# CIS565-Fall-2014/Project3-Pathtracer

Measured on AMD Instinct MI355X. Metric: ray-bounces/sec, higher is better.
Workload: dtype f32

## Files before the change

### project3-pathtracer_amd/csrc/pt_bounce.h

```cpp
#pragma once
#include <stdlib.h>

#include "pt_internal.h"

namespace pt {
using namespace ptd;

static constexpr uint32_t DEAD = 0xFFFFFFFFu;
#ifndef PT_DEBUG_PAIR
#define PT_DEBUG_PAIR 0
#endif
#ifndef PT_DEBUG_PHASE
#define PT_DEBUG_PHASE 0
#endif
#ifndef PT_DEBUG_BVH
#define PT_DEBUG_BVH 0
#endif
#ifndef PT_DEBUG_SPAN
#define PT_DEBUG_SPAN 0
#endif
static constexpr bool DEBUG_SPAN = PT_DEBUG_SPAN != 0;
#ifndef PT_DEBUG_BOUNDS
#define PT_DEBUG_BOUNDS 0
#endif
// ... 3 lines not shown
static constexpr bool DEBUG_PHASE = PT_DEBUG_PHASE == 1;
static constexpr bool DEBUG_PHASE2 = PT_DEBUG_PHASE == 2;
template <bool FIRST> __device__ __forceinline__ constexpr bool LANE_BUDGET() { return FIRST ? PT_DEBUG_PHASE == 3 : PT_DEBUG_PHASE == 2; }
static constexpr bool DEBUG_BVH = PT_DEBUG_BVH != 0;
static constexpr int MAXSLOT = 16;
static constexpr uint32_t SLOT_SHIFT = 27;
static constexpr uint32_t PIX_MASK = (1u << SLOT_SHIFT) - 1u;

typedef const __attribute__((address_space(4))) uint32_t *const_u32_ptr;
typedef float v4f __attribute__((ext_vector_type(4)));
typedef float v2f __attribute__((ext_vector_type(2)));
template <class V> __device__ __forceinline__ void nt_store(V v, V *p)
{
#if defined(PT_NO_NT)
    *p = v;
#else
    __builtin_nontemporal_store(v, p);
#endif
}
template <class V> __device__ __forceinline__ V nt_load(const V *p)
{
#if defined(PT_NO_NT)
    return *p;
#else
    return __builtin_nontemporal_load(p);
#endif
}

__device__ __forceinline__ bool dbgInRange(const KParams &p, int code, unsigned long long v, unsigned long long lim)
{
    if (!DEBUG_BOUNDS || v < lim) return true;
    if (atomicCAS(&p.st->dbg[0], 0ull, (unsigned long long)code) == 0ull) { p.st->dbg[1] = v; p.st->dbg[2] = lim; p.st->dbg[4] = blockIdx.x; p.st->dbg[5] = threadIdx.x; }
    return false;
}

__device__ __forceinline__ Prim load_prim_scalar(const Prim *prims, int g)
{
    Prim r;
    const_u32_ptr q = (const_u32_ptr)(uintptr_t)(prims + g);
    uint32_t *dst = reinterpret_cast<uint32_t *>(&r);
#pragma unroll
    for (int k = 0; k < 32; ++k) dst[k] = q[k];
    return r;
}

struct PrimPad : Prim { uint32_t pad_lds[4]; };
static_assert(sizeof(PrimPad) == 144, "PrimPad must be 144 B");
template <class PR> __device__ __forceinline__ constexpr uint32_t faceStride() { return (uint32_t)(sizeof(PR) / 16); }

struct Hit {
    f3 p, n;
    uint32_t material;
    uint32_t prim;
    float t;
    bool any;
    uint32_t self_ok;
    unsigned long long dbg0, dbg1;
    unsigned long long dbg2, dbg3;
};

enum { GEOM_SCALAR = 0, GEOM_LDS = 1, GEOM_QUEUE = 2, GEOM_BVH = 3, GEOM_PAIR = 4, GEOM_WALK_PAIR = 5, GEOM_WALK4 = 6,
       GEOM_WALK4G = 7 };

__device__ __forceinline__ bool waveMissesBound(const Prim &P, f3 o, f3 d)
{
    const f3 oc = o - mk(P.cx, P.cy, P.cz);
// ... 1545 lines not shown
                        q = (q < 0.05f) ? 0.05f : ((q > 1.0f) ? 1.0f : q);
                        if (u01_of(minstd_jump(s0, MINSTD_A4)) >= q) alive = false;
                        else T = mk(T.x / q, T.y / q, T.z / q);
                    }
                    if (NEE) pix = (pix & 0x7FFFFFFFu) | (diffuse ? 0x80000000u : 0u);
                    }
                }
            }
        }
        if (NEE) {
            const uint64_t wmask = __ballot(want_shadow);
            if (wmask != 0ull) {
                shadow_count += (uint32_t)__popcll(wmask);
                Hit hs;
                if (MOTION && GEOM == GEOM_PAIR) {
                    hs = nearestHit<GEOM, false, true>(p, s_prims, s_nodes + (PAIR_BOX_BYTES / 16) * p.nG, wq, so, sd, want_shadow, (uint32_t)lane, 0xFFFFFFFFu, mt);
                } else if (MOTION) {
                    hs.any = false; hs.material = 0; hs.prim = 0; hs.t = 0.0f; hs.p = mk(0, 0, 0); hs.n = mk(0, 0, 0);
                    if (want_shadow) hs = nearestHitMotion(p, so, sd, mt);
                } else {
                    hs = nearestHit<GEOM, false>(p, s_prims, (GEOM == GEOM_PAIR) ? s_nodes + (PAIR_BOX_BYTES / 16) * p.nG : s_nodes, wq, so, sd, want_shadow, (uint32_t)lane);
                }
                if (want_shadow && hs.any && hs.prim == lprim) {
                    const float tol = 1e-3f * ((ldist > 1.0f) ? ldist : 1.0f);
                    if (fabsf(hs.t - ldist) <= tol) L = L + Ld;
                }
            }
            if (valid && (L.x != 0.0f || L.y != 0.0f || L.z != 0.0f)) {
                float4 *lp = reinterpret_cast<float4 *>(p.lbuf) + ((size_t)((pix >> SLOT_SHIFT) & (uint32_t)(MAXSLOT - 1)) * npix + (size_t)(pix & PIX_MASK));
                if (!dbgInRange(p, 6, (unsigned long long)((pix >> SLOT_SHIFT) & (uint32_t)(MAXSLOT - 1)) * npix + (pix & PIX_MASK), (unsigned long long)npix * st->nslot)) lp = reinterpret_cast<float4 *>(p.lbuf);
                float4 e = *lp;
                if (__float_as_uint(e.w) != serial) e = make_float4(0.0f, 0.0f, 0.0f, 0.0f);
                *lp = make_float4(e.x + L.x, e.y + L.y, e.z + L.z, __uint_as_float(serial));
            }
        } else if (valid && !alive && (L.x != 0.0f || L.y != 0.0f || L.z != 0.0f)) {
            float4 *lp = reinterpret_cast<float4 *>(p.lbuf) + ((size_t)(pix >> SLOT_SHIFT) * npix + (size_t)(pix & PIX_MASK));
            if (!dbgInRange(p, 7, (unsigned long long)(pix >> SLOT_SHIFT) * npix + (pix & PIX_MASK), (unsigned long long)npix * st->nslot)) lp = reinterpret_cast<float4 *>(p.lbuf);
            nt_store((v4f){L.x, L.y, L.z, __uint_as_float(serial)}, reinterpret_cast<v4f *>(lp));
        }

        const unsigned long long c3 = (DEBUG_PHASE || PT_DEBUG_PHASE == 2 || PT_DEBUG_PHASE == 3) ? __builtin_amdgcn_s_memtime() : 0ull;
        if (DEBUG_PHASE) { ph[0] += c1 - tc0; ph[1] += c2 - c1; ph[2] += c3 - c2; ph[4] += 1; }
        if (LANE_BUDGET<FIRST>()) { ph[0] += c1 - tc0; ph[1] += c2 - c1; ph[2] += c3 - c2; ph[4] += 1; ph5 += h.dbg0 + h.dbg2; ph6 += h.dbg1; }
        if (LANE_BUDGET<FIRST>() && GEOM == GEOM_PAIR) {
            lb_nbsdf = (uint32_t)__popcll(__ballot(did_bsdf));
            const unsigned long long res = (c2 - c1) - h.dbg0 - h.dbg1 - h.dbg2;
            lbud[0] += c1 - tc0;  lbud[1] += (c1 - tc0) * lb_nvalid;
            lbud[2] += h.dbg0;    lbud[3] += h.dbg0 * lb_nvalid;
            lbud[4] += h.dbg2;
            lbud[5] += h.dbg1;    lbud[6] += h.dbg3;
            lbud[7] += res;       lbud[8] += res * lb_nhit;
            lbud[9] += c3 - c2;   lbud[10] += (c3 - c2) * lb_nbsdf;
            lbud[13] += 1;        lbud[14] += lb_nvalid;
        }
        if (RESIDENT) {
            if (valid && !alive) atomicAdd(&s_term[cb], 1u);
            valid = alive;
            lb = (cb + 1u) | (leaves_outside ? ((h.prim + 1u) << 8) : 0u);
            if (DEBUG_PHASE2 && GEOM == GEOM_PAIR) { const unsigned long long c4 = __builtin_amdgcn_s_memtime() - c3; lbud[11] += c4; lbud[12] += c4 * (unsigned long long)__popcll(__ballot(alive)); }
            continue;
        }
        if (last) continue;

        if (COMPACT != 0) {
            const uint64_t mask = __ballot(alive);
            const uint32_t rank = __builtin_amdgcn_mbcnt_hi((uint32_t)(mask >> 32),
                                                            __builtin_amdgcn_mbcnt_lo((uint32_t)mask, 0u));
            const uint32_t wtot = (uint32_t)__popcll(mask);
            uint32_t dst;
            if (COMPACT == 1 || NW == 1) {
                uint32_t b = 0;
// ... 161 lines not shown
```

### project3-pathtracer_amd/csrc/pt_context.hip

```cpp
#include <math.h>
#include <stdarg.h>
#include <stdio.h>
#include <stdlib.h>
#include <string.h>

#include <algorithm>
#include <string>
#include <vector>

#include "pt_internal.h"
#include "pt_scene.h"

#ifndef PT_RESIDENT_DEFAULT
#define PT_RESIDENT_DEFAULT 1
#endif
#ifndef PT_REFILL_MIN_DEFAULT
#define PT_REFILL_MIN_DEFAULT 8
#endif

namespace {
thread_local std::string g_last_error;
}

int pt::fail(int code, const char *fmt, ...)
// ... 54 lines not shown
    pt::KParams kps[PT_MAX_SEQUENCES];
    int nseq = 1;
    hipStream_t seq_stream[PT_MAX_SEQUENCES] = {};
    hipEvent_t seq_acc[PT_MAX_SEQUENCES] = {};
    hipEvent_t seq_fork = nullptr;
    pt::LaunchCfg cfg;
    ptd::Prim *d_prims = nullptr;
    float *d_mats = nullptr;
    float *d_ro_eye = nullptr;
    float *d_face_n = nullptr;
    float *d_box_eye = nullptr;
    std::vector<float> h_box_eye;
    std::vector<ptd::BvhNode> h_bvh;
    std::vector<float> h_boxes;
    uint32_t *d_span_off = nullptr, *d_span_list = nullptr;
    size_t span_off_cap = 0, span_list_cap = 0;
    uint32_t *d_span_mask = nullptr;
    size_t span_mask_cap = 0;
    float *d_box_world = nullptr;
    float *d_slab_n = nullptr;
    pt::LightRec *d_lights = nullptr;
    float *d_knots = nullptr, *d_knot_cam = nullptr;
    int *d_light_tris = nullptr;
    float *d_light_cdf = nullptr;
    ptd::BvhNode *d_bvh = nullptr;
    float *d_bvh4 = nullptr;
    float *d_image_own = nullptr;
    float *d_image_bound = nullptr;
    size_t image_bytes = 0, image_cap = 0;
    void *d_pool = nullptr;
    size_t pool_cap = 0;
    float *d_lbuf = nullptr;
    size_t lbuf_cap = 0;
    unsigned long long batches_stamped = 0;
    int batch = 1;
    pt::IterState *d_state = nullptr;
    bool image_valid = false;

    hipGraph_t graph[PT_MAX_SEQUENCES + 1] = {};
    hipGraphExec_t graph_exec[PT_MAX_SEQUENCES + 1] = {};

    std::vector<std::pair<hipEvent_t, hipEvent_t>> timers;
    double gpu_ms = 0.0;
    unsigned long long bounce_launches = 0;
};

namespace {

void drop_graph(pt_ctx *c)
{
    for (int q = 0; q <= PT_MAX_SEQUENCES; ++q) {
        if (c->graph_exec[q]) { (void)hipGraphExecDestroy(c->graph_exec[q]); c->graph_exec[q] = nullptr; }
        if (c->graph[q]) { (void)hipGraphDestroy(c->graph[q]); c->graph[q] = nullptr; }
    }
}

hipError_t sync_all_streams(pt_ctx *c)
{
    hipError_t first = hipStreamSynchronize(c->stream);
    for (int sq = 1; sq < PT_MAX_SEQUENCES; ++sq)
        if (c->seq_stream[sq]) {
            const hipError_t e = hipStreamSynchronize(c->seq_stream[sq]);
            if (first == hipSuccess) first = e;
        }
    return first;
}
// ... 879 lines not shown
    if (per_cu < 1) return fail(PT_ERR_HIP, "occupancy query failed for workgroup=%d (%s)", cfg.workgroup,
                                hipGetErrorString(hipGetLastError()));
    {
        const long long fit = (160LL * 1024) / ((long long)lds + 1300);
        if (fit >= 1 && per_cu > (int)fit) per_cu = (int)fit;
    }
    int cap = 6 * 256 / cfg.workgroup;
    if (cap < 1) cap = 1;
    if (getenv("PT_MAX_WG_PER_CU") && atoi(getenv("PT_MAX_WG_PER_CU")) > 0) cap = atoi(getenv("PT_MAX_WG_PER_CU"));
    if (per_cu > cap) per_cu = cap;
    int batch = o.batch == 0 ? pt::PT_MAX_BATCH : o.batch;
    while (batch > 1 && (long long)npix * batch > (1LL << 28)) --batch;
    if (npix >= (1 << 27)) return fail(PT_ERR_INVALID, "tile of %d pixels too large (pixel index must fit 27 bits)", npix);
    c->batch = batch;
    k.nslot = batch;
    const long long nrays = (long long)npix * batch;
    const long long want = (nrays + cfg.workgroup - 1) / cfg.workgroup;
    long long grid = (long long)c->cu_count * per_cu;
    if (grid > want) grid = want;
    if (grid < 1) grid = 1;
    cfg.grid = (int)grid;
    if (cfg.resident && !pt::bounce_resident_available(cfg)) cfg.resident = 0;
    cfg.slab = slab_wanted();
    if (!cfg.slab) k.slab_mask = 0u;
    if (getenv("PT_DEBUG_CLOCK"))
        fprintf(stderr, "[ptamd] launch: geom %d, workgroup %d, %zu B LDS, %d workgroups/CU, grid %d, batch %d, resident paths %d (refill at %d free lanes)\n", cfg.geom, cfg.workgroup,
                lds, per_cu, cfg.grid, batch, cfg.resident, k.refill_min);

    int nseq = o.sequences == 0 ? 2 : o.sequences;
    if (o.sequences == 0 && getenv("PT_SEQUENCES") && atoi(getenv("PT_SEQUENCES")) >= 1 && atoi(getenv("PT_SEQUENCES")) <= PT_MAX_SEQUENCES)
        nseq = atoi(getenv("PT_SEQUENCES"));
    c->nseq = nseq;
    const size_t lbuf_bytes = ((size_t)nrays * 4 * sizeof(float) + 255) & ~(size_t)255;

    k.span_mask = nullptr;
    k.span_off = nullptr;
    k.span_list = nullptr;
    const bool spans_ok = k.eye_cull && !(k.lens_radius > 0.0f) && npix / 64 <= (1 << 21);
    const bool want_mask = spans_ok && !cfg.motion && cfg.geom == 4 && k.nG <= 32 && k.ntri == 0 && c->h_box_eye.size() >= (size_t)k.nG * 8;
    const bool want_lists = spans_ok && npix % 64 == 0 && (cfg.geom == 6 || cfg.geom == 7) && c->h_boxes.size() >= (size_t)k.nG * 6 && k.nG <= 65536;
    if (want_mask || want_lists) {
        const int nspan = (npix + 63) / 64;
        const double ex = k.eye[0], ey = k.eye[1], ez = k.eye[2];
        const double eye3[3] = {ex, ey, ez};
        const double vw[3] = {(double)k.M[0] - ex, (double)k.M[1] - ey, (double)k.M[2] - ez};
        auto gpix = [&](uint32_t pl) -> uint32_t {
            if (k.strip_span == 0u) return pl + k.pix_offset;
            const uint32_t j = pl / k.strip_span;
            return pl + k.strip_span * (j * (k.strip_world - 1u) + k.strip_rank);
        };
        auto dirOf = [&](double sx, double sy, double *o3) {
            for (int a = 0; a < 3; ++a) o3[a] = vw[a] + (1.0 - 2.0 * sx) * (double)k.H[a] + (1.0 - 2.0 * sy) * (double)k.V[a];
        };
        double sx_margin, sy_margin;
        {
            double big = 0.0, lh = 0.0, lv = 0.0;
            for (int a = 0; a < 3; ++a) {
                big = std::max(big, fabs(eye3[a]) + fabs(vw[a]) + fabs((double)k.H[a]) + fabs((double)k.V[a]));
                lh += (double)k.H[a] * (double)k.H[a]; lv += (double)k.V[a] * (double)k.V[a];
            }
            const double err = 3.0 * 1.1920929e-7 * big * 1.7320508;
            sx_margin = lh > 0.0 ? err / (2.0 * sqrt(lh)) : 1e30;
            sy_margin = lv > 0.0 ? err / (2.0 * sqrt(lv)) : 1e30;
        }
        const bool ray_grid_ok = sx_margin < 1.0 && sy_margin < 1.0;
        struct Frustum { double nrm[4][3], cc[3], lcc; bool planes_ok, narrow; };
// ... 128 lines not shown
            }
        }
    }

    {
        const long long nw = cfg.workgroup / 64;
        const long long total_waves = (long long)cfg.grid * nw;
        const long long chunks = (nrays + 63) / 64 + pt::NSHARD;
        const long long rounds = (chunks + total_waves - 1) / total_waves;
        long long writers = total_waves;
        if (k.nshard > 1) writers = (total_waves + k.nshard - 1) / k.nshard;
        long long segcap = writers * rounds * 64;
        const long long npad = (nrays + 63) & ~63LL;
        if (k.nshard == 1 || segcap > npad) segcap = npad;
        k.segcap = (uint32_t)segcap;
    }
    const size_t slots = (size_t)k.segcap * (size_t)k.nshard;
    const size_t one = slots * (16 + 16 + 8);
    for (;;) {
        hipError_t e = hipSuccess;
        if (c->lbuf_cap < lbuf_bytes * (size_t)nseq) {
            if (c->d_lbuf) (void)hipFree(c->d_lbuf);
            c->d_lbuf = nullptr; c->lbuf_cap = 0;
            e = hipMalloc((void **)&c->d_lbuf, lbuf_bytes * (size_t)nseq);
            if (e == hipSuccess) {
                c->lbuf_cap = lbuf_bytes * (size_t)nseq;
                HIP_TRY(hipMemsetAsync(c->d_lbuf, 0, c->lbuf_cap, c->stream));
                HIP_TRY(hipStreamSynchronize(c->stream));
                for (uint32_t sq = 0; sq < (uint32_t)PT_MAX_SEQUENCES; ++sq)
                    HIP_TRY(hipMemcpy(&c->d_state[sq].serial, &sq, sizeof sq, hipMemcpyHostToDevice));
                c->batches_stamped = 0;
            } else c->d_lbuf = nullptr;
        }
        if (e == hipSuccess && c->pool_cap < 2 * one * (size_t)nseq) {
            if (c->d_pool) (void)hipFree(c->d_pool);
            c->d_pool = nullptr; c->pool_cap = 0;
            e = hipMalloc(&c->d_pool, 2 * one * (size_t)nseq);
            if (e == hipSuccess) c->pool_cap = 2 * one * (size_t)nseq;
            else c->d_pool = nullptr;
        }
        if (e == hipSuccess) break;
        (void)hipGetLastError();
        if (nseq > 1) { nseq = 1; c->nseq = 1; continue; }
        c->dirty = true;
        return fail(PT_ERR_OOM, "device memory: %zu B of ray pools + %zu B of radiance planes per launch sequence (%s)", 2 * one, lbuf_bytes,
                    hipGetErrorString(e));
    }
    k.lbuf = c->d_lbuf;
    for (int sq = 0; sq < PT_MAX_SEQUENCES; ++sq) {
        pt::KParams &ks = c->kps[sq];
        ks = k;
        if (sq >= nseq) continue;
        for (int q = 0; q < 2; ++q) {
            unsigned char *base = (unsigned char *)c->d_pool + (size_t)(2 * sq + q) * one;
            ks.pool[q].a = (float4 *)base;
            ks.pool[q].b = (float4 *)(base + slots * 16);
            ks.pool[q].c = (float2 *)(base + slots * 32);
        }
        ks.lbuf = (float *)((unsigned char *)c->d_lbuf + (size_t)sq * lbuf_bytes);
        ks.st = c->d_state + sq;
    }
    k = c->kps[0];
    if (getenv("PT_DEBUG_CLOCK")) fprintf(stderr, "[ptamd] launch sequences in flight: %d\n", nseq);

    c->dirty = false;
    return PT_OK;
}

int bounce_launches_per_batch(const pt_ctx *c) { return c->cfg.resident ? 2 : c->kp.depth; }

int book_batch_serials(pt_ctx *c, unsigned long long nb)
{
    static const unsigned long long serial_budget =
        (getenv("PT_SERIAL_BUDGET") && atoll(getenv("PT_SERIAL_BUDGET")) > 0) ? (unsigned long long)atoll(getenv("PT_SERIAL_BUDGET")) : (1ull << 29);
    if (c->batches_stamped + nb > serial_budget) {
        HIP_TRY(sync_all_streams(c));
        HIP_TRY(hipMemset(c->d_lbuf, 0, c->lbuf_cap));
        for (uint32_t sq = 0; sq < (uint32_t)PT_MAX_SEQUENCES; ++sq)
            HIP_TRY(hipMemcpy(&c->d_state[sq].serial, &sq, sizeof sq, hipMemcpyHostToDevice));
        c->batches_stamped = 0;
    }
    c->batches_stamped += nb;
    return PT_OK;
}

int enqueue_batch(pt_ctx *c, hipStream_t s, hipEvent_t *ev, int sq = 0, bool with_accumulate = true)
{
    const pt::KParams &kp = c->kps[sq];
    HIP_TRY(pt::launch_iter_begin(s, kp.st, kp.npix, kp.depth, c->cfg.compact));
    const int launches = bounce_launches_per_batch(c);
    for (int b = 0; b < launches; ++b) {
        if (ev) HIP_TRY(hipEventRecord(ev[2 * b], s));
        HIP_TRY(pt::launch_bounce(s, kp, c->cfg, b));
        if (ev) HIP_TRY(hipEventRecord(ev[2 * b + 1], s));
    }
    if (with_accumulate) HIP_TRY(pt::launch_accumulate(s, kp.image, kp.lbuf, kp.st, kp.npix));
    return PT_OK;
}

void batch_schedule(int iter_count, int batch, int *n, int *q, int *r)
{
    *n = (iter_count + batch - 1) / batch;
    *q = iter_count / *n;
    *r = iter_count % *n;
}

float lerp1(float a, float b, float t) { return a + (b - a) * t; }
pt_vec3 lerp3(pt_vec3 a, pt_vec3 b, float t) { return {lerp1(a.x, b.x, t), lerp1(a.y, b.y, t), lerp1(a.z, b.z, t)}; }

void drop_slices(pt_ctx *c)
{
    for (pt_ctx *k : c->slice_ctx) pt_destroy(k);
    c->slice_ctx.clear();
}

int build_slices(pt_ctx *c)
{
    if (!c->motion_dirty) return PT_OK;
    drop_slices(c);
    const int n = c->motion_slices;
    for (int k = 0; k < n; ++k) {
        pt_ctx *ch = nullptr;
        int rc = pt_create(c->device, &ch);
        if (rc != PT_OK) return rc;
        c->slice_ctx.push_back(ch);
        const float t = ((float)k + 0.5f) / (float)n;
        std::vector<pt_static_geom> g = c->geoms;
        for (size_t i = 0; i < g.size(); ++i) {
            const pt_static_geom &a = c->geoms[i], &b = c->geoms_next[i];
// ... 17 lines not shown
                while (a1 < c->tri_geom.size() && c->tri_geom[a1] == c->tri_geom[a0]) ++a1;
                ms.push_back(pt_mesh{c->tri_geom[a0], (int)(a1 - a0), c->tri_obj.data() + 9 * a0});
                a0 = a1;
            }
            rc = pt_set_meshes(ch, ms.data(), (int)ms.size());
        }
        if (rc == PT_OK) rc = pt_set_camera(ch, &cam);
        if (rc != PT_OK) return rc;
    }
    c->motion_dirty = false;
    return PT_OK;
}

int render_batch_ordered(pt_ctx *c, hipStream_t ss, int iter_first, int count, hipEvent_t wait_ev, hipEvent_t done_ev)
{
    int rc = configure(c);
    if (rc != PT_OK) return rc;
    if (count < 1 || count > c->batch) return fail(PT_ERR_INVALID, "render_batch_ordered: %d iterations (batch %d)", count, c->batch);
    rc = book_batch_serials(c, 1ull);
    if (rc != PT_OK) return rc;
    if (c->opt.use_graph && !c->graph_exec[0]) {
        HIP_TRY(hipStreamBeginCapture(ss, hipStreamCaptureModeThreadLocal));
        rc = enqueue_batch(c, ss, nullptr, 0, false);
        hipError_t ce = hipStreamEndCapture(ss, &c->graph[0]);
        if (rc != PT_OK) { drop_graph(c); return rc; }
        if (ce != hipSuccess) { drop_graph(c); return fail(PT_ERR_HIP, "hipStreamEndCapture: %s", hipGetErrorString(ce)); }
        HIP_TRY(hipGraphInstantiate(&c->graph_exec[0], c->graph[0], nullptr, nullptr, 0));
    }
    HIP_TRY(pt::launch_iter_set(ss, c->d_state, (uint32_t)iter_first, (uint32_t)count, 0u, 0u, 1u));
    if (c->opt.use_graph) HIP_TRY(hipGraphLaunch(c->graph_exec[0], ss));
    else { rc = enqueue_batch(c, ss, nullptr, 0, false); if (rc != PT_OK) return rc; }
    if (wait_ev) HIP_TRY(hipStreamWaitEvent(ss, wait_ev, 0));
    const pt::KParams &ks = c->kps[0];
    HIP_TRY(pt::launch_accumulate(ss, ks.image, ks.lbuf, ks.st, ks.npix));
    HIP_TRY(pt::launch_iter_fold(ss, c->d_state, c->kp.depth));
    if (done_ev) HIP_TRY(hipEventRecord(done_ev, ss));
    c->bounce_launches += (unsigned long long)bounce_launches_per_batch(c);
    c->image_valid = true;
    return PT_OK;
}

}

extern "C" {

const char *pt_last_error(void) { return g_last_error.c_str(); }
const char *pt_version(void) { return "ptamd 0.1 (gfx950, abi 2)"; }
int pt_abi_version(void) { return PT_ABI_VERSION; }
size_t pt_options_size(void) { return sizeof(pt_options); }

int pt_strip_local_rows(int height, int strip_rows, int world, int rank)
{
    if (height < 1 || strip_rows < 1 || world < 1 || rank < 0 || rank >= world) return 0;
    const long long nstrips = ((long long)height + strip_rows - 1) / strip_rows;
    long long rows = 0;
    for (long long k = rank; k < nstrips; k += world) {
        const long long left = (long long)height - k * strip_rows;
        rows += left < strip_rows ? left : strip_rows;
    }
    return (int)rows;
}

int pt_strip_global_row(int strip_rows, int world, int rank, int local_row)
{
    if (strip_rows < 1 || world < 1 || rank < 0 || rank >= world || local_row < 0) return -1;
    const int j = local_row / strip_rows, w = local_row % strip_rows;
    return (j * world + rank) * strip_rows + w;
// ... 55 lines not shown
            pt_destroy(c);
            return fail(PT_ERR_HIP, "cannot initialise the iteration state");
        }
    *out = c;
    return PT_OK;
}

void pt_destroy(pt_ctx *c)
{
    if (!c) return;
    drop_slices(c);
    (void)hipSetDevice(c->device);
    if (c->stream) (void)sync_all_streams(c);
    drop_graph(c);
    for (auto &t : c->timers) { (void)hipEventDestroy(t.first); (void)hipEventDestroy(t.second); }
    if (c->d_prims) (void)hipFree(c->d_prims);
    if (c->d_mats) (void)hipFree(c->d_mats);
    if (c->d_ro_eye) (void)hipFree(c->d_ro_eye);
    if (c->d_face_n) (void)hipFree(c->d_face_n);
    if (c->d_box_eye) (void)hipFree(c->d_box_eye);
    if (c->d_span_mask) (void)hipFree(c->d_span_mask);
    if (c->d_box_world) (void)hipFree(c->d_box_world);
    if (c->d_slab_n) (void)hipFree(c->d_slab_n);
    if (c->d_lights) (void)hipFree(c->d_lights);
    if (c->d_light_tris) (void)hipFree(c->d_light_tris);
    if (c->d_light_cdf) (void)hipFree(c->d_light_cdf);
    if (c->d_knots) (void)hipFree(c->d_knots);
    if (c->d_knot_cam) (void)hipFree(c->d_knot_cam);
    if (c->d_bvh) (void)hipFree(c->d_bvh);
    if (c->d_bvh4) (void)hipFree(c->d_bvh4);
    if (c->d_image_own) (void)hipFree(c->d_image_own);
    if (c->d_pool) (void)hipFree(c->d_pool);
    if (c->d_lbuf) (void)hipFree(c->d_lbuf);
    if (c->d_state) (void)hipFree(c->d_state);
    if (c->d_span_off) (void)hipFree(c->d_span_off);
    if (c->d_span_list) (void)hipFree(c->d_span_list);
    for (int q = 1; q < PT_MAX_SEQUENCES; ++q)
        if (c->seq_stream[q]) { (void)hipStreamSynchronize(c->seq_stream[q]); (void)hipStreamDestroy(c->seq_stream[q]); }
    for (int q = 0; q < PT_MAX_SEQUENCES; ++q)
        if (c->seq_acc[q]) (void)hipEventDestroy(c->seq_acc[q]);
    if (c->seq_fork) (void)hipEventDestroy(c->seq_fork);
    if (c->own_stream) (void)hipStreamDestroy(c->own_stream);
    delete c;
}

int pt_set_options(pt_ctx *c, const pt_options *o)
{
    if (!c || !o) return fail(PT_ERR_INVALID, "pt_set_options: NULL argument");
    if (o->depth < 1 || o->depth > PT_MAX_DEPTH) return fail(PT_ERR_INVALID, "depth %d not in 1..%d", o->depth, PT_MAX_DEPTH);
    const int wg = o->workgroup;
    if (!(wg == 0 || wg == 64 || wg == 128 || wg == 256 || wg == 512 || wg == 1024))
        return fail(PT_ERR_INVALID, "workgroup %d not one of 0,64,128,256,512,1024", wg);
    if (o->geom_path < 0 || o->geom_path > 8) return fail(PT_ERR_INVALID, "geom_path %d not in 0..8", o->geom_path);
    if (o->row_begin < 0 || o->row_end < o->row_begin) return fail(PT_ERR_INVALID, "tile rows [%d,%d)", o->row_begin, o->row_end);
    if (o->strip_rows < 0 || (o->strip_rows > 0 && (o->strip_world < 1 || o->strip_rank < 0 || o->strip_rank >= o->strip_world)))
        return fail(PT_ERR_INVALID, "strips: rows %d, rank %d of %d", o->strip_rows, o->strip_rank, o->strip_world);
    if (o->strip_rows > 0 && (o->row_begin != 0 || o->row_end != 0))
        return fail(PT_ERR_INVALID, "strip tiles and a row band [%d,%d) exclude each other", o->row_begin, o->row_end);
    if (o->batch < 0 || o->batch > pt::PT_MAX_BATCH) return fail(PT_ERR_INVALID, "batch %d not in 0..%d", o->batch, pt::PT_MAX_BATCH);
    if (o->compaction < 0 || o->compaction > 2) return fail(PT_ERR_INVALID, "compaction %d not 0, 1 or 2", o->compaction);
    if (o->direct_light < 0 || o->direct_light > 1) return fail(PT_ERR_INVALID, "direct_light %d not 0 or 1", o->direct_light);
    if (o->absorption < 0 || o->absorption > 1) return fail(PT_ERR_INVALID, "absorption %d not 0 or 1", o->absorption);
    if (o->scatter < 0 || o->scatter > 1) return fail(PT_ERR_INVALID, "scatter %d not 0 or 1", o->scatter);
    if (!(o->lens_radius >= 0.0f) || (o->lens_radius > 0.0f && !(o->focal_distance > 0.0f)))
        return fail(PT_ERR_INVALID, "lens radius %g / focal distance %g", (double)o->lens_radius, (double)o->focal_distance);
    if (o->motion_per_ray < 0 || o->motion_per_ray > 1) return fail(PT_ERR_INVALID, "motion_per_ray %d not 0 or 1", o->motion_per_ray);
// ... 260 lines not shown
            if (ce != hipSuccess) { drop_graph(c); return fail(PT_ERR_HIP, "hipStreamEndCapture: %s", hipGetErrorString(ce)); }
            HIP_TRY(hipGraphInstantiate(&c->graph_exec[gs], c->graph[gs], nullptr, nullptr, 0));
        }
    }
    rc = book_batch_serials(c, (unsigned long long)nb);
    if (rc != PT_OK) return rc;
    if (c->timers.size() >= 1024) { rc = fold_timers(c); if (rc != PT_OK) return rc; }
    hipEvent_t e0, e1;
    HIP_TRY(hipEventCreateWithFlags(&e0, hipEventDisableSystemFence));
    HIP_TRY(hipEventCreateWithFlags(&e1, hipEventDisableSystemFence));
    c->timers.emplace_back(e0, e1);
    HIP_TRY(hipEventRecord(e0, s));

    auto forked = [&]() -> int {
        if (nseq > 1) {
            HIP_TRY(hipEventRecord(c->seq_fork, s));
            for (int sq = 1; sq < nseq; ++sq) HIP_TRY(hipStreamWaitEvent(c->seq_stream[sq], c->seq_fork, 0));
        }
        for (int sq = 0; sq < nseq; ++sq)
            HIP_TRY(pt::launch_iter_set(c->seq_stream[sq], c->d_state + sq, (uint32_t)iter_first, (uint32_t)q, (uint32_t)r, (uint32_t)sq, (uint32_t)nseq));
        for (int i = 0; i < nb; ++i) {
            const int sq = i % nseq;
            hipStream_t ss = c->seq_stream[sq];
            if (c->opt.use_graph) {
                const int gs = own_acc ? sq : PT_MAX_SEQUENCES;
                HIP_TRY(hipGraphLaunch(c->graph_exec[gs], ss));
            } else {
                const int rc2 = enqueue_batch(c, ss, nullptr, sq, !own_acc);
                if (rc2 != PT_OK) return rc2;
            }
            if (own_acc) {
                if (i > 0) HIP_TRY(hipStreamWaitEvent(ss, c->seq_acc[(i - 1) % nseq], 0));
                const pt::KParams &ks = c->kps[sq];
                HIP_TRY(pt::launch_accumulate(ss, ks.image, ks.lbuf, ks.st, ks.npix));
                HIP_TRY(hipEventRecord(c->seq_acc[sq], ss));
            }
        }
        for (int sq = 0; sq < nseq; ++sq) HIP_TRY(pt::launch_iter_fold(c->seq_stream[sq], c->d_state + sq, c->kp.depth));
        if (nseq > 1) {
            for (int sq = 1; sq < nseq; ++sq) {
                HIP_TRY(hipEventRecord(c->seq_acc[sq], c->seq_stream[sq]));
                HIP_TRY(hipStreamWaitEvent(s, c->seq_acc[sq], 0));
            }
        }
        HIP_TRY(hipEventRecord(e1, s));
        return PT_OK;
    };
    rc = forked();
    if (rc != PT_OK) {
        (void)sync_all_streams(c);
        c->image_valid = false;
        return rc;
    }
    c->bounce_launches += (unsigned long long)nb * (unsigned long long)bounce_launches_per_batch(c);
    c->image_valid = true;
    return PT_OK;
}

int pt_get_launch_info(pt_ctx *c, pt_launch_info *out)
{
    if (!c || !out) return fail(PT_ERR_INVALID, "pt_get_launch_info: NULL argument");
    int rc = configure(c);
    if (rc != PT_OK) return rc;
    memset(out, 0, sizeof *out);
    out->geom_path = c->cfg.geom + 1;
    out->workgroup = c->cfg.workgroup;
    out->grid = c->cfg.grid;
// ... 231 lines not shown
```

### project3-pathtracer_amd/csrc/pt_internal.h

```cpp
#pragma once
#include <hip/hip_runtime.h>
#include <stdint.h>

#include "../../include/pt_abi.h"
#include "pt_device.h"

namespace pt {

struct RayPool {
    float4 *a;
    float4 *b;
    float2 *c;
};

static constexpr int NSHARD = 32;
static constexpr int PT_MAX_BATCH = 16;
static constexpr int CNT_STRIDE = 32;
__host__ __device__ constexpr int cnt_index(int bounce, int shard) { return (bounce * NSHARD + shard) * CNT_STRIDE; }

struct IterState {
    uint32_t iter;
    uint32_t nslot;
    uint32_t sched_q, sched_r, sched_j;
    uint32_t sched_first, sched_stride;
// ... 18 lines not shown
    float lens_radius, focal_distance;
    int W;
    int row_begin;
    int npix;
    uint32_t pix_offset;
    int nG, nM;
    int depth;
    int rr_start;
    uint32_t seed;
    const ptd::Prim *prims;
    const ptd::BvhNode *bvh;
    int nnodes;
    const float *bvh4;
    int nnodes4;
    int wdepth;
    int ntri;
    int nbig;
    int big[16];
    const float *face_n;
    const float *ro_eye;
    int eye_cull;
    const float *box_world;
    const float *box_eye;
    const float *slab_n;
    uint32_t slab_mask;
    const uint32_t *span_off;
    const uint32_t *span_list;
    const uint32_t *span_mask;
    const float *mats;
    float *image;
    int cull;
    int nslot;
    float *lbuf;
    int nshard;
    uint32_t segcap;
    IterState *st;
    RayPool pool[2];
    uint32_t strip_span;
    uint32_t strip_rows, strip_world, strip_rank;
    uint32_t strip_magic;
    uint32_t strip_shift;
    uint32_t w_magic;
    uint32_t w_shift;
    int absorption;
    int scatter;
    int nlights;
    const LightRec *lights;
    const int *light_tris;
    const float *light_cdf;
    int ngeoms;
    const float *knots;
    const float *knot_cam;
    int nknots;
    float tan_x, tan_y;
    int refill_min;
};

struct LaunchCfg {
    int workgroup;
    int grid;
    int geom;
    int compact;
    int nee;
    int media;
    int motion;
    int resident;
    int slab;
};

hipError_t launch_iter_set(hipStream_t s, IterState *st, uint32_t iter_first, uint32_t q, uint32_t r, uint32_t j0, uint32_t stride);
hipError_t launch_iter_begin(hipStream_t s, IterState *st, int npix, int depth, int compact);
hipError_t launch_accumulate(hipStream_t s, float *image, const float *lbuf, const IterState *st, int npix);
hipError_t launch_iter_fold(hipStream_t s, IterState *st, int depth);
hipError_t launch_bounce(hipStream_t s, const KParams &p, const LaunchCfg &cfg, int bounce);
hipError_t launch_send_image_to_pbo(hipStream_t s, pt_uchar4 *pbo, const float *image, int npix);
hipError_t launch_selftest_math(hipStream_t s, unsigned long long *out3);
hipError_t launch_device_kat(hipStream_t s, int op, const float *in, float *out, int n_out);
int fail(int code, const char *fmt, ...) __attribute__((format(printf, 2, 3)));

size_t bounce_lds_bytes(const KParams &p, const LaunchCfg &cfg);
int bounce_max_blocks_per_cu(const KParams &p, const LaunchCfg &cfg);
bool bounce_resident_available(const LaunchCfg &cfg);

}
```

### project3-pathtracer_amd/csrc/pt_kernels.hip

```cpp
#include <stdlib.h>

#include <algorithm>

#include "pt_bounce.h"

namespace pt {

__global__ __launch_bounds__(256) void k_selftest_math(unsigned long long *out)
{
    const uint64_t stride = (uint64_t)gridDim.x * 256u;
    unsigned long long bad0 = 0, bad1 = 0, bad2 = 0;
    for (uint64_t i = (uint64_t)blockIdx.x * 256u + threadIdx.x; i < (1ull << 32); i += stride) {
        const float x = __uint_as_float((uint32_t)i);
        const float a = sqrtf(x), b = sqrt_rn(x);
        if (__float_as_uint(a) != __float_as_uint(b) && !(a != a && b != b)) bad0++;
        const float c = 1.0f / x, d = rcp_rn(x);
        if (__float_as_uint(c) != __float_as_uint(d) && !(c != c && d != d)) bad1++;
        const float e = 1.0f / sqrtf(x), f = rsqrt_rn(x), g = rsqrt_near_one(x);
        if (__float_as_uint(e) != __float_as_uint(f) && !(e != e && f != f)) bad2++;
        if (__float_as_uint(e) != __float_as_uint(g) && !(e != e && g != g)) bad2++;
        const uint32_t sd = (uint32_t)i, md = sd % 2147483647u;
        if (minstd_seed(sd) != (md == 0u ? 1u : md)) bad2++;
    }
    if (bad0) atomicAdd(&out[0], bad0);
// ... 95 lines not shown
    st->nslot = 0u;
    st->sched_q = q;
    st->sched_r = r;
    st->sched_j = j0;
    st->sched_first = iter_first;
    st->sched_stride = stride;
}

__global__ void k_iter_begin(IterState *st, uint32_t npix, int depth, int compact)
{
    const int b = threadIdx.x;
    const uint32_t j = st->sched_j;
    const uint32_t nslot = st->sched_q + (j < st->sched_r ? 1u : 0u);
    const uint32_t iter = st->sched_first + j * st->sched_q + (j < st->sched_r ? j : st->sched_r);
    __syncthreads();
    if (b <= depth) {
        unsigned long long sum = 0;
        for (int sh = 0; sh < NSHARD; ++sh) {
            sum += st->counts[cnt_index(b, sh)];
            st->counts[cnt_index(b, sh)] = (b == 0 && sh == 0 && compact) ? npix * nslot : 0u;
        }
        if (b < depth) st->live_in[b] += sum;
    }
    if (b < NSHARD) st->draw[b * CNT_STRIDE] = 0u;
    if (b == 0) {
        st->serial += (uint32_t)PT_MAX_SEQUENCES;
        st->iter = iter;
        st->nslot = nslot;
        st->sched_j = j + st->sched_stride;
        st->iterations += nslot;
    }
}

__global__ __launch_bounds__(256) void k_accumulate(float *image, const float4 *lbuf, const IterState *st, int npix)
{
    const uint32_t iter0 = st->iter, serial = st->serial;
    const int nslot = (int)st->nslot;
    for (int i = blockIdx.x * 256 + threadIdx.x; i < npix; i += gridDim.x * 256) {
        float r = image[3 * i], g = image[3 * i + 1], b = image[3 * i + 2];
        float4 L[PT_MAX_BATCH];
#pragma unroll
        for (int k = 0; k < PT_MAX_BATCH; ++k)
            if (k < nslot) {
                const v4f e = __builtin_nontemporal_load(reinterpret_cast<const v4f *>(lbuf + (size_t)k * (size_t)npix + (size_t)i));
                L[k] = make_float4(e.x, e.y, e.z, e.w);
            }
#pragma unroll
        for (int k = 0; k < PT_MAX_BATCH; ++k) {
            if (k < nslot) {
                const bool have = __float_as_uint(L[k].w) == serial;
                const float lr = have ? L[k].x : 0.0f, lg = have ? L[k].y : 0.0f, lb = have ? L[k].z : 0.0f;
                const uint32_t it = iter0 + (uint32_t)k;
                const float fi = (float)it, fim1 = (float)(it - 1u);
                r = (it == 1u) ? lr : (r * fim1 + lr) / fi;
                g = (it == 1u) ? lg : (g * fim1 + lg) / fi;
                b = (it == 1u) ? lb : (b * fim1 + lb) / fi;
            }
        }
        image[3 * i] = r;
        image[3 * i + 1] = g;
        image[3 * i + 2] = b;
    }
}

__global__ void k_iter_fold(IterState *st, int depth)
{
    const int b = threadIdx.x;
    if (b <= depth) {
        unsigned long long sum = 0;
        for (int sh = 0; sh < NSHARD; ++sh) {
            sum += st->counts[cnt_index(b, sh)];
            st->counts[cnt_index(b, sh)] = 0u;
        }
        if (b < depth) st->live_in[b] += sum;
    }
}

__global__ __launch_bounds__(256) void k_send_image_to_pbo(pt_uchar4 *pbo, const float *image, int npix)
{
    for (int i = blockIdx.x * 256 + threadIdx.x; i < npix; i += gridDim.x * 256) {
        float r = image[3 * i] * 255.0f, g = image[3 * i + 1] * 255.0f, b = image[3 * i + 2] * 255.0f;
        if (r > 255) r = 255;
        if (g > 255) g = 255;
        if (b > 255) b = 255;
        pt_uchar4 o;
        o.x = (unsigned char)r;
        o.y = (unsigned char)g;
        o.z = (unsigned char)b;
        o.w = 0;
        pbo[i] = o;
    }
// ... 59 lines not shown
            hipFuncSetAttribute(f0, hipFuncAttributeMaxDynamicSharedMemorySize, (int)lds) != hipSuccess)
            return 0;
    }
    if (hipOccupancyMaxActiveBlocksPerMultiprocessor(&nb, fn, cfg.workgroup, bounce_lds_bytes(p, cfg)) != hipSuccess)
        return 0;
    return nb;
}

hipError_t launch_bounce(hipStream_t s, const KParams &p, const LaunchCfg &cfg, int bounce)
{
    LaunchCfg lc = cfg;
    if (bounce == 0) lc.resident = 0;
    const void *fn = select_bounce(lc, bounce == 0);
    if (!fn) return hipErrorInvalidValue;
    KParams pc = p;
    int b = bounce;
    void *args[] = {(void *)&pc, (void *)&b};
    return hipLaunchKernel(fn, dim3((unsigned)cfg.grid), dim3((unsigned)cfg.workgroup), args,
                           bounce_lds_bytes(p, lc), s);
}

hipError_t launch_iter_set(hipStream_t s, IterState *st, uint32_t iter_first, uint32_t q, uint32_t r, uint32_t j0, uint32_t stride)
{
    hipLaunchKernelGGL(k_iter_set, dim3(1), dim3(1), 0, s, st, iter_first, q, r, j0, stride);
    return hipGetLastError();
}

hipError_t launch_iter_begin(hipStream_t s, IterState *st, int npix, int depth, int compact)
{
    hipLaunchKernelGGL(k_iter_begin, dim3(1), dim3(128), 0, s, st, (uint32_t)npix, depth, compact != 0 ? 1 : 0);
    return hipGetLastError();
}

hipError_t launch_accumulate(hipStream_t s, float *image, const float *lbuf, const IterState *st, int npix)
{
    int grid = (npix + 255) / 256;
    if (grid > 16384) grid = 16384;
    if (grid < 1) grid = 1;
    hipLaunchKernelGGL(k_accumulate, dim3(grid), dim3(256), 0, s, image, reinterpret_cast<const float4 *>(lbuf), st, npix);
    return hipGetLastError();
}

hipError_t launch_iter_fold(hipStream_t s, IterState *st, int depth)
{
    hipLaunchKernelGGL(k_iter_fold, dim3(1), dim3(128), 0, s, st, depth);
    return hipGetLastError();
}

hipError_t launch_send_image_to_pbo(hipStream_t s, pt_uchar4 *pbo, const float *image, int npix)
{
    int grid = (npix + 255) / 256;
    if (grid > 4096) grid = 4096;
    if (grid < 1) grid = 1;
    hipLaunchKernelGGL(k_send_image_to_pbo, dim3(grid), dim3(256), 0, s, pbo, image, npix);
    return hipGetLastError();
}

}
```

Baseline: 54290.

## Track written light slots per pixel to skip empty loads in accumulate

Adds a per-pixel bitmask, set atomically by the bounce kernel whenever a slot's radiance buffer entry is written. The accumulate kernel then gathers only the marked slots instead of loading every batch slot, and clears the mask afterwards. This is meant to cut memory traffic in accumulation, since many pixel/slot pairs receive no light. In exchange it adds an atomic OR on every radiance write in the bounce kernel, extra mask memory, and more branchy control flow in accumulate.

```diff
diff --git a/profiles/r05/call_tail.py b/profiles/r05/call_tail.py
--- /dev/null
+++ b/profiles/r05/call_tail.py
@@ -0,0 +1,22 @@
+#!/usr/bin/env python3
+import csv, os, sys
+sys.path.insert(0, os.path.join(os.path.dirname(os.path.abspath(__file__)), '..'))
+from timeline import short
+for path in sys.argv[1:]:
+    rows = sorted(csv.DictReader(open(path)), key=lambda r: int(r["Start_Timestamp"]))
+    rows = [r for r in rows if short(r["Kernel_Name"]) in ("camera", "resident", "k_accumulate", "accumulate", "iter_begin", "iter_set", "iter_fold")]
+    calls, cur = [], []
+    for r in rows:
+        n = short(r["Kernel_Name"])
+        if n == "iter_set" and cur and short(cur[-1]["Kernel_Name"]) != "iter_set":
+            calls.append(cur); cur = []
+        cur.append(r)
+    calls.append(cur)
+    print("==", path, len(calls), "calls")
+    for c in calls[-6:]:
+        t0 = int(c[0]["Start_Timestamp"]); t1 = max(int(r["End_Timestamp"]) for r in c)
+        res = [int(r["End_Timestamp"]) for r in c if short(r["Kernel_Name"]) == "resident"]
+        acc = [(int(r["Start_Timestamp"]), int(r["End_Timestamp"])) for r in c if short(r["Kernel_Name"]) == "accumulate"]
+        nres = len(res)
+        print(f"  call: {nres} resident, span {(t1 - t0)/1e3:8.1f} us, after last resident {(t1 - max(res))/1e3 if res else 0:7.1f} us, "
+              f"accumulates (start,end rel. to last resident end) {[((a-max(res))/1e3, (b-max(res))/1e3) for a,b in acc][-3:] if res else acc}")
diff --git a/project3-pathtracer_amd/csrc/pt_bounce.h b/project3-pathtracer_amd/csrc/pt_bounce.h
--- a/project3-pathtracer_amd/csrc/pt_bounce.h
+++ b/project3-pathtracer_amd/csrc/pt_bounce.h
@@ -59,6 +59,13 @@
     if (!DEBUG_BOUNDS || v < lim) return true;
     if (atomicCAS(&p.st->dbg[0], 0ull, (unsigned long long)code) == 0ull) { p.st->dbg[1] = v; p.st->dbg[2] = lim; p.st->dbg[4] = blockIdx.x; p.st->dbg[5] = threadIdx.x; }
     return false;
+}
+
+__device__ __forceinline__ void mark_slot(const KParams &p, uint32_t px, uint32_t slot)
+{
+    uint32_t *m = p.smask + px;
+    if (!dbgInRange(p, 2, (unsigned long long)px, (unsigned long long)p.npix)) m = p.smask;
+    __hip_atomic_fetch_or(m, 1u << slot, __ATOMIC_RELAXED, __HIP_MEMORY_SCOPE_AGENT);
 }
 
 __device__ __forceinline__ Prim load_prim_scalar(const Prim *prims, int g)
@@ -1670,11 +1677,13 @@
                 float4 e = *lp;
                 if (__float_as_uint(e.w) != serial) e = make_float4(0.0f, 0.0f, 0.0f, 0.0f);
                 *lp = make_float4(e.x + L.x, e.y + L.y, e.z + L.z, __uint_as_float(serial));
+                mark_slot(p, pix & PIX_MASK, (pix >> SLOT_SHIFT) & (uint32_t)(MAXSLOT - 1));
             }
         } else if (valid && !alive && (L.x != 0.0f || L.y != 0.0f || L.z != 0.0f)) {
             float4 *lp = reinterpret_cast<float4 *>(p.lbuf) + ((size_t)(pix >> SLOT_SHIFT) * npix + (size_t)(pix & PIX_MASK));
             if (!dbgInRange(p, 7, (unsigned long long)(pix >> SLOT_SHIFT) * npix + (pix & PIX_MASK), (unsigned long long)npix * st->nslot)) lp = reinterpret_cast<float4 *>(p.lbuf);
             nt_store((v4f){L.x, L.y, L.z, __uint_as_float(serial)}, reinterpret_cast<v4f *>(lp));
+            mark_slot(p, pix & PIX_MASK, pix >> SLOT_SHIFT);
         }
 
         const unsigned long long c3 = (DEBUG_PHASE || PT_DEBUG_PHASE == 2 || PT_DEBUG_PHASE == 3) ? __builtin_amdgcn_s_memtime() : 0ull;
diff --git a/project3-pathtracer_amd/csrc/pt_context.hip b/project3-pathtracer_amd/csrc/pt_context.hip
--- a/project3-pathtracer_amd/csrc/pt_context.hip
+++ b/project3-pathtracer_amd/csrc/pt_context.hip
@@ -110,6 +110,8 @@
     size_t pool_cap = 0;
     float *d_lbuf = nullptr;
     size_t lbuf_cap = 0;
+    uint32_t *d_smask = nullptr;
+    size_t smask_cap = 0;
     unsigned long long batches_stamped = 0;
     int batch = 1;
     pt::IterState *d_state = nullptr;
@@ -1055,6 +1057,7 @@
         nseq = atoi(getenv("PT_SEQUENCES"));
     c->nseq = nseq;
     const size_t lbuf_bytes = ((size_t)nrays * 4 * sizeof(float) + 255) & ~(size_t)255;
+    const size_t smask_bytes = ((size_t)npix * sizeof(uint32_t) + 255) & ~(size_t)255;
 
     k.span_mask = nullptr;
     k.span_off = nullptr;
@@ -1249,6 +1252,16 @@
                 c->batches_stamped = 0;
             } else c->d_lbuf = nullptr;
         }
+        if (e == hipSuccess && c->smask_cap < smask_bytes * (size_t)nseq) {
+            if (c->d_smask) (void)hipFree(c->d_smask);
+            c->d_smask = nullptr; c->smask_cap = 0;
+            e = hipMalloc((void **)&c->d_smask, smask_bytes * (size_t)nseq);
+            if (e == hipSuccess) {
+                c->smask_cap = smask_bytes * (size_t)nseq;
+                HIP_TRY(hipMemsetAsync(c->d_smask, 0, c->smask_cap, c->stream));
+                HIP_TRY(hipStreamSynchronize(c->stream));
+            } else c->d_smask = nullptr;
+        }
         if (e == hipSuccess && c->pool_cap < 2 * one * (size_t)nseq) {
             if (c->d_pool) (void)hipFree(c->d_pool);
             c->d_pool = nullptr; c->pool_cap = 0;
@@ -1264,6 +1277,7 @@
                     hipGetErrorString(e));
     }
     k.lbuf = c->d_lbuf;
+    k.smask = c->d_smask;
     for (int sq = 0; sq < PT_MAX_SEQUENCES; ++sq) {
         pt::KParams &ks = c->kps[sq];
         ks = k;
@@ -1275,6 +1289,7 @@
             ks.pool[q].c = (float2 *)(base + slots * 32);
         }
         ks.lbuf = (float *)((unsigned char *)c->d_lbuf + (size_t)sq * lbuf_bytes);
+        ks.smask = (uint32_t *)((unsigned char *)c->d_smask + (size_t)sq * smask_bytes);
         ks.st = c->d_state + sq;
     }
     k = c->kps[0];
@@ -1293,6 +1308,7 @@
     if (c->batches_stamped + nb > serial_budget) {
         HIP_TRY(sync_all_streams(c));
         HIP_TRY(hipMemset(c->d_lbuf, 0, c->lbuf_cap));
+        HIP_TRY(hipMemset(c->d_smask, 0, c->smask_cap));
         for (uint32_t sq = 0; sq < (uint32_t)PT_MAX_SEQUENCES; ++sq)
             HIP_TRY(hipMemcpy(&c->d_state[sq].serial, &sq, sizeof sq, hipMemcpyHostToDevice));
         c->batches_stamped = 0;
@@ -1311,7 +1327,7 @@
         HIP_TRY(pt::launch_bounce(s, kp, c->cfg, b));
         if (ev) HIP_TRY(hipEventRecord(ev[2 * b + 1], s));
     }
-    if (with_accumulate) HIP_TRY(pt::launch_accumulate(s, kp.image, kp.lbuf, kp.st, kp.npix));
+    if (with_accumulate) HIP_TRY(pt::launch_accumulate(s, kp.image, kp.lbuf, kp.smask, kp.st, kp.npix));
     return PT_OK;
 }
 
@@ -1395,7 +1411,7 @@
     else { rc = enqueue_batch(c, ss, nullptr, 0, false); if (rc != PT_OK) return rc; }
     if (wait_ev) HIP_TRY(hipStreamWaitEvent(ss, wait_ev, 0));
     const pt::KParams &ks = c->kps[0];
-    HIP_TRY(pt::launch_accumulate(ss, ks.image, ks.lbuf, ks.st, ks.npix));
+    HIP_TRY(pt::launch_accumulate(ss, ks.image, ks.lbuf, ks.smask, ks.st, ks.npix));
     HIP_TRY(pt::launch_iter_fold(ss, c->d_state, c->kp.depth));
     if (done_ev) HIP_TRY(hipEventRecord(done_ev, ss));
     c->bounce_launches += (unsigned long long)bounce_launches_per_batch(c);
@@ -1517,6 +1533,7 @@
     if (c->d_image_own) (void)hipFree(c->d_image_own);
     if (c->d_pool) (void)hipFree(c->d_pool);
     if (c->d_lbuf) (void)hipFree(c->d_lbuf);
+    if (c->d_smask) (void)hipFree(c->d_smask);
     if (c->d_state) (void)hipFree(c->d_state);
     if (c->d_span_off) (void)hipFree(c->d_span_off);
     if (c->d_span_list) (void)hipFree(c->d_span_list);
@@ -1843,7 +1860,7 @@
             if (own_acc) {
                 if (i > 0) HIP_TRY(hipStreamWaitEvent(ss, c->seq_acc[(i - 1) % nseq], 0));
                 const pt::KParams &ks = c->kps[sq];
-                HIP_TRY(pt::launch_accumulate(ss, ks.image, ks.lbuf, ks.st, ks.npix));
+                HIP_TRY(pt::launch_accumulate(ss, ks.image, ks.lbuf, ks.smask, ks.st, ks.npix));
                 HIP_TRY(hipEventRecord(c->seq_acc[sq], ss));
             }
         }
diff --git a/project3-pathtracer_amd/csrc/pt_internal.h b/project3-pathtracer_amd/csrc/pt_internal.h
--- a/project3-pathtracer_amd/csrc/pt_internal.h
+++ b/project3-pathtracer_amd/csrc/pt_internal.h
@@ -74,6 +74,7 @@
     int cull;
     int nslot;
     float *lbuf;
+    uint32_t *smask;
     int nshard;
     uint32_t segcap;
     IterState *st;
@@ -112,7 +113,7 @@
 
 hipError_t launch_iter_set(hipStream_t s, IterState *st, uint32_t iter_first, uint32_t q, uint32_t r, uint32_t j0, uint32_t stride);
 hipError_t launch_iter_begin(hipStream_t s, IterState *st, int npix, int depth, int compact);
-hipError_t launch_accumulate(hipStream_t s, float *image, const float *lbuf, const IterState *st, int npix);
+hipError_t launch_accumulate(hipStream_t s, float *image, const float *lbuf, uint32_t *smask, const IterState *st, int npix);
 hipError_t launch_iter_fold(hipStream_t s, IterState *st, int depth);
 hipError_t launch_bounce(hipStream_t s, const KParams &p, const LaunchCfg &cfg, int bounce);
 hipError_t launch_send_image_to_pbo(hipStream_t s, pt_uchar4 *pbo, const float *image, int npix);
diff --git a/project3-pathtracer_amd/csrc/pt_kernels.hip b/project3-pathtracer_amd/csrc/pt_kernels.hip
--- a/project3-pathtracer_amd/csrc/pt_kernels.hip
+++ b/project3-pathtracer_amd/csrc/pt_kernels.hip
@@ -151,31 +151,53 @@
     }
 }
 
-__global__ __launch_bounds__(256) void k_accumulate(float *image, const float4 *lbuf, const IterState *st, int npix)
+static constexpr int ACC_GATHER = 4;
+
+__global__ __launch_bounds__(256) void k_accumulate(float *image, const float4 *lbuf, uint32_t *smask, const IterState *st, int npix)
 {
     const uint32_t iter0 = st->iter, serial = st->serial;
     const int nslot = (int)st->nslot;
+    const uint32_t live = (1u << nslot) - 1u;
     for (int i = blockIdx.x * 256 + threadIdx.x; i < npix; i += gridDim.x * 256) {
+        const uint32_t m0 = smask[i];
+        uint32_t m = m0 & live;
+        int ks[ACC_GATHER];
+        float4 e[ACC_GATHER];
+        auto gather = [&]() {
+#pragma unroll
+            for (int j = 0; j < ACC_GATHER; ++j) {
+                ks[j] = m ? __builtin_ctz(m) : 32;
+                m &= m - 1u;
+                e[j] = make_float4(0.0f, 0.0f, 0.0f, 0.0f);
+                if (ks[j] < 32) {
+                    const v4f v = __builtin_nontemporal_load(reinterpret_cast<const v4f *>(lbuf + (size_t)ks[j] * (size_t)npix + (size_t)i));
+                    e[j] = make_float4(v.x, v.y, v.z, v.w);
+                }
+            }
+        };
+        gather();
+        __asm__ volatile("" ::: "memory");
         float r = image[3 * i], g = image[3 * i + 1], b = image[3 * i + 2];
-        float4 L[PT_MAX_BATCH];
+        int k = 0;
+        for (;;) {
+            const int kend = m ? ks[ACC_GATHER - 1] + 1 : nslot;
+            for (; k < kend; ++k) {
+                float4 L = make_float4(0.0f, 0.0f, 0.0f, 0.0f);
 #pragma unroll
-        for (int k = 0; k < PT_MAX_BATCH; ++k)
-            if (k < nslot) {
-                const v4f e = __builtin_nontemporal_load(reinterpret_cast<const v4f *>(lbuf + (size_t)k * (size_t)npix + (size_t)i));
-                L[k] = make_float4(e.x, e.y, e.z, e.w);
-            }
-#pragma unroll
-        for (int k = 0; k < PT_MAX_BATCH; ++k) {
-            if (k < nslot) {
-                const bool have = __float_as_uint(L[k].w) == serial;
-                const float lr = have ? L[k].x : 0.0f, lg = have ? L[k].y : 0.0f, lb = have ? L[k].z : 0.0f;
+                for (int j = 0; j < ACC_GATHER; ++j)
+                    if (k == ks[j]) L = e[j];
+                const bool have = __float_as_uint(L.w) == serial;
+                const float lr = have ? L.x : 0.0f, lg = have ? L.y : 0.0f, lb = have ? L.z : 0.0f;
                 const uint32_t it = iter0 + (uint32_t)k;
                 const float fi = (float)it, fim1 = (float)(it - 1u);
                 r = (it == 1u) ? lr : (r * fim1 + lr) / fi;
                 g = (it == 1u) ? lg : (g * fim1 + lg) / fi;
                 b = (it == 1u) ? lb : (b * fim1 + lb) / fi;
             }
+            if (!m) break;
+            gather();
         }
+        if (m0 != 0u) smask[i] = 0u;
         image[3 * i] = r;
         image[3 * i + 1] = g;
         image[3 * i + 2] = b;
@@ -301,12 +323,12 @@
     return hipGetLastError();
 }
 
-hipError_t launch_accumulate(hipStream_t s, float *image, const float *lbuf, const IterState *st, int npix)
+hipError_t launch_accumulate(hipStream_t s, float *image, const float *lbuf, uint32_t *smask, const IterState *st, int npix)
 {
     int grid = (npix + 255) / 256;
     if (grid > 16384) grid = 16384;
     if (grid < 1) grid = 1;
-    hipLaunchKernelGGL(k_accumulate, dim3(grid), dim3(256), 0, s, image, reinterpret_cast<const float4 *>(lbuf), st, npix);
+    hipLaunchKernelGGL(k_accumulate, dim3(grid), dim3(256), 0, s, image, reinterpret_cast<const float4 *>(lbuf), smask, st, npix);
     return hipGetLastError();
 }
 
```

New measurement: 55070 (median of 6 runs). +1.4%, better.
